# mourisl/Rcorrector

Measured on AMD Instinct MI355X. Metric: corrected reads/sec (150 bp, k=23), higher is better.
Workload: dtype u8/int32/u64

## Files before the change

### include/rcorrector_amd.h

```cpp
#ifndef RCORRECTOR_AMD_H
#define RCORRECTOR_AMD_H

#include <stddef.h>
#include <stdint.h>

#ifdef __cplusplus
extern "C" {
#endif

typedef struct rc_ctx rc_ctx;

typedef enum {
    RC_STATUS_OK = 0,
    RC_STATUS_ARG = -1,
    RC_STATUS_HIP = -2,
    RC_STATUS_IO = -3,
    RC_STATUS_STATE = -4,
    RC_STATUS_NOMEM = -5,
    RC_STATUS_NOSPACE = -6
} rc_status;

typedef struct {
    int device;
    int k;
// ... 189 lines not shown

typedef struct {
    int mode;
    uint32_t n_reads;
    uint64_t nbytes;
    int32_t max_read_len;
    uint8_t *d_seq;
    const uint8_t *d_qual;
    const uint32_t *d_off;
    int32_t *d_ret, *d_l, *d_m, *d_h;
} rc_device_batch;
int rc_correct_device(rc_ctx *ctx, const rc_device_batch *b);
int rc_strong_threshold_device(rc_ctx *ctx, const uint8_t *d_seq, const uint32_t *d_off, uint32_t n_reads,
                               uint64_t nbytes, int32_t max_read_len, int32_t *d_strong);
int rc_strong_threshold_read(rc_ctx *ctx, const char *seq, int32_t *strong);
int rc_correct_read(rc_ctx *ctx, char *seq, const char *qual, int32_t pair_strong_threshold, int32_t *ret);
int rc_kmer_info_read(rc_ctx *ctx, const char *seq, int32_t *l, int32_t *m, int32_t *h);
int rc_probe_device(rc_ctx *ctx, const uint8_t *d_seq, uint64_t nbytes, int32_t *d_counts);
int rc_sync(rc_ctx *ctx);

int rc_profile_enable(rc_ctx *ctx, int on);
int rc_profile_correct_counters(rc_ctx *ctx, uint64_t *reads_listed, uint64_t *gather_rounds, uint64_t *bucket_requests);
int rc_profile_read_rounds(rc_ctx *ctx, int32_t *d_rounds);
int rc_profile_get(rc_ctx *ctx, int kernel, double *total_ms, uint64_t *launches);
int rc_profile_reset(rc_ctx *ctx);

int rc_selftest_get_bound(rc_ctx *ctx, const int32_t *c, size_t n, double error_rate, int32_t *out_int, double *out_dbl);

int rc_debug_routes(rc_ctx *ctx, uint8_t *cls_out, uint8_t *cand_out, uint64_t *runs_out, uint32_t n);

int rc_summary(const rc_ctx *ctx, uint64_t *total_reads, uint64_t *total_corrections);

#ifdef __cplusplus
}
#endif
#endif
```

### rcorrector_amd/binding.py

```python
import ctypes as C
import os
import subprocess

import numpy as np

HERE = os.path.dirname(os.path.abspath(__file__))
CSRC = os.path.join(HERE, "csrc")

ABI_SYMBOLS = [
    "rc_create", "rc_destroy", "rc_last_error", "rc_device_numa_node", "rc_device_memory",
    "rc_table_build", "rc_table_build_device", "rc_table_load_jfdump",
    "rc_table_count_begin", "rc_table_count_add", "rc_table_count_add_device", "rc_table_count_finish",
    "rc_table_count_keep", "rc_table_count_arenas", "rc_table_count_release", "rc_table_count_park", "rc_table_count_finish_sharded", "rc_submit_resident", "rc_wait_resident",
    "rc_table_count_reads_device", "rc_table_write_jfdump", "rc_table_share", "rc_table_replicate", "rc_table_replicate_async", "rc_table_lookup", "rc_table_export", "rc_table_digest", "rc_table_layout", "rc_table_stats",
    "rc_table_count_spectrum", "rc_table_spectrum",
    "rc_recount_begin", "rc_recount_add", "rc_recount_add_device", "rc_recount_follow", "rc_recount_finish",
    "rc_change_report_begin", "rc_change_report_get", "rc_change_report_end",
    "rc_weak_profile_device", "rc_weak_profile_into",
    "rc_dup_census_begin", "rc_dup_census_get", "rc_dup_census_end", "rc_read_keys_device", "rc_dup_census_merge",
    "rc_trust_profile_device", "rc_trust_profile_begin", "rc_trust_profile_get", "rc_trust_profile_end",
    "rc_mate_overlap_device", "rc_mate_overlap_begin", "rc_mate_overlap_get", "rc_mate_overlap_end",
    "rc_estimate_error_rate", "rc_bad_quality_from_hist", "rc_set_run_params", "rc_set_quality_bits", "rc_pack_quality_bits",
    "rc_correct_batch", "rc_set_slot_lanes", "rc_runtime_prepare", "rc_submit", "rc_wait", "rc_host_alloc", "rc_host_free", "rc_host_register", "rc_host_unregister", "rc_correct_batch_traced", "rc_correct_device", "rc_strong_threshold_device", "rc_probe_device", "rc_sync",
    "rc_strong_threshold_read", "rc_correct_read", "rc_kmer_info_read",
    "rc_pack_bases", "rc_submit_packed", "rc_wait_packed", "rc_apply_fixes",
    "rc_profile_enable", "rc_profile_get", "rc_profile_reset", "rc_profile_correct_counters", "rc_profile_read_rounds", "rc_selftest_get_bound", "rc_debug_routes", "rc_summary",
]


class RcorrectorError(RuntimeError):
    pass


def library_path():
    return os.environ.get("RC_LIB") or os.path.join(HERE, "librcorrector_amd.so")


def build_library(quiet=True):
    subprocess.run(["make", "-C", CSRC, "-j4", "all"], check=True,
                   stdout=subprocess.DEVNULL if quiet else None)
    return library_path()


class _Config(C.Structure):
    _fields_ = [("device", C.c_int), ("k", C.c_int), ("max_fix_per_k", C.c_int)]


class _Batch(C.Structure):
    _fields_ = [("mode", C.c_int), ("n", C.c_size_t),
# ... 182 lines not shown
    L.rc_correct_batch.argtypes = [vp, C.POINTER(_Batch)]
    L.rc_submit.argtypes = [vp, C.POINTER(_Batch), C.c_int]
    L.rc_wait.argtypes = [vp, C.c_int]
    L.rc_host_alloc.argtypes = [vp, sz, C.POINTER(C.c_void_p)]
    L.rc_host_free.argtypes = [vp, vp]
    L.rc_correct_device.argtypes = [vp, C.POINTER(_DeviceBatch)]
    L.rc_probe_device.argtypes = [vp, vp, C.c_uint64, vp]
    L.rc_strong_threshold_device.argtypes = [vp, vp, vp, C.c_uint32, C.c_uint64, C.c_int32, vp]
    L.rc_sync.argtypes = [vp]
    L.rc_strong_threshold_read.argtypes = [vp, C.c_char_p, C.POINTER(C.c_int32)]
    L.rc_correct_read.argtypes = [vp, C.c_char_p, C.c_char_p, C.c_int32, C.POINTER(C.c_int32)]
    L.rc_kmer_info_read.argtypes = [vp, C.c_char_p, C.POINTER(C.c_int32), C.POINTER(C.c_int32), C.POINTER(C.c_int32)]
    L.rc_pack_bases.restype = sz
    L.rc_pack_bases.argtypes = [vp, sz, sz, vp, vp, vp, sz]
    L.rc_submit_packed.argtypes = [vp, C.POINTER(_PackedBatch), C.c_int]
    L.rc_wait_packed.argtypes = [vp, C.c_int]
    L.rc_apply_fixes.restype = None
    L.rc_apply_fixes.argtypes = [vp, vp, vp, sz]
    L.rc_profile_enable.argtypes = [vp, C.c_int]
    L.rc_profile_get.argtypes = [vp, C.c_int, C.POINTER(C.c_double), C.POINTER(C.c_uint64)]
    L.rc_profile_reset.argtypes = [vp]
    L.rc_profile_correct_counters.argtypes = [vp, C.POINTER(C.c_uint64), C.POINTER(C.c_uint64), C.POINTER(C.c_uint64)]
    L.rc_profile_read_rounds.argtypes = [vp, vp]
    L.rc_selftest_get_bound.argtypes = [vp, vp, sz, C.c_double, vp, vp]
    L.rc_debug_routes.argtypes = [vp, vp, vp, vp, C.c_uint32]
    L.rc_summary.argtypes = [vp, C.POINTER(C.c_uint64), C.POINTER(C.c_uint64)]
    _lib = L
    return L


def runtime_prepare(hw_queues=16):
    return load_library().rc_runtime_prepare(int(hw_queues))


def pack_reads(seqs):
    lens = np.fromiter((len(s) for s in seqs), dtype=np.int64, count=len(seqs))
    off = np.zeros(len(seqs) + 1, dtype=np.uint32)
    np.cumsum(lens + 1, out=off[1:])
    if seqs:
        arena = np.frombuffer(b"\0".join(seqs) + b"\0", dtype=np.uint8).copy()
    else:
        arena = np.zeros(0, np.uint8)
    return arena, off


def unpack_reads(arena, off):
# ... 443 lines not shown

    def kmer_info_read(self, seq):
        l, m, h = C.c_int32(0), C.c_int32(0), C.c_int32(0)
        self._ck(self._L.rc_kmer_info_read(self._h, bytes(seq), C.byref(l), C.byref(m), C.byref(h)))
        return l.value, m.value, h.value

    def probe_device(self, d_seq, nbytes, d_counts):
        self._ck(self._L.rc_probe_device(self._h, _ptr(d_seq), nbytes, _ptr(d_counts)))

    def sync(self):
        self._ck(self._L.rc_sync(self._h))

    def profile(self, on=True):
        self._ck(self._L.rc_profile_enable(self._h, int(on)))

    def profile_correct_counters(self):
        a, b, c = C.c_uint64(0), C.c_uint64(0), C.c_uint64(0)
        self._ck(self._L.rc_profile_correct_counters(self._h, C.byref(a), C.byref(b), C.byref(c)))
        return a.value, b.value, c.value

    def profile_read_rounds(self, d_rounds=None):
        self._ck(self._L.rc_profile_read_rounds(self._h, None if d_rounds is None else d_rounds.data_ptr()))

    def profile_reset(self):
        self._ck(self._L.rc_profile_reset(self._h))

    def profile_get(self, kernel):
        ms, n = C.c_double(0), C.c_uint64(0)
        self._ck(self._L.rc_profile_get(self._h, kernel, C.byref(ms), C.byref(n)))
        return ms.value, n.value

    def selftest_get_bound(self, c, error_rate):
        c = np.ascontiguousarray(c, dtype=np.int32)
        oi = np.zeros(len(c), dtype=np.int32)
        od = np.zeros(len(c), dtype=np.float64)
        self._ck(self._L.rc_selftest_get_bound(self._h, c.ctypes.data, len(c), error_rate, oi.ctypes.data, od.ctypes.data))
        return oi, od

    def debug_routes(self, n):
        cls, cand, runs = np.zeros(n, np.uint8), np.zeros(n, np.uint8), np.zeros(n, np.uint64)
        self._ck(self._L.rc_debug_routes(self._h, cls.ctypes.data, cand.ctypes.data, runs.ctypes.data, n))
        return cls, cand, runs

    def summary(self):
        a, b = C.c_uint64(0), C.c_uint64(0)
        self._ck(self._L.rc_summary(self._h, C.byref(a), C.byref(b)))
# ... 2 lines not shown
```

### rcorrector_amd/csrc/rc_api.hip

```cpp
#include "rc_api_internal.h"
#include <mutex>

static thread_local char g_create_err[512];

void rc_set_error(rc_ctx *ctx, const char *fmt, ...)
{
    va_list ap;
    va_start(ap, fmt);
    vsnprintf(ctx ? ctx->err : g_create_err, 512, fmt, ap);
    va_end(ap);
}

int rc_dbuf_reserve(rc_ctx *ctx, rc_dbuf *b, size_t bytes)
{
    if (bytes <= b->bytes) return RC_OK;
    if (b->p) {
        RC_CHECK_HIP(ctx, hipStreamSynchronize(ctx->stream));
        (void)hipFree(b->p);
        b->p = nullptr;
        b->bytes = 0;
    }
    size_t want = bytes + bytes / 8 + 256;
    RC_CHECK_HIP(ctx, hipMalloc(&b->p, want));
    b->bytes = want;
// ... 99 lines not shown
        ln->is_lane = true;
        ln->lane_parent = ctx;
    }
    if (refresh) {
        ln->d_buckets = ctx->d_buckets;
        ln->buckets_borrowed = true;
        ln->nb_home = ctx->nb_home;
        ln->layout = ctx->layout;
        ln->ext = ctx->ext;
        ln->nb_alloc = ctx->nb_alloc;
        ln->n_entries = ctx->n_entries;
        ln->table_bytes = ctx->table_bytes;
        ln->filter_words = ctx->filter_words;
        ln->filter_kind = ctx->filter_kind;
        ln->filter_all = ctx->filter_all;
        ln->P = ctx->P;
        ln->params_set = ctx->params_set;
        ln->qual_bits = ctx->qual_bits;
        ln->kept.arenas = ctx->kept.arenas;
        ln->profile = ctx->profile;
        ln->phase_prof = ctx->phase_prof;
        ln->phase_prof_print = ctx->phase_prof_print;
        ln->rounds_out = ctx->rounds_out;
    }
    ctx->slot_home[slot] = ln;
    return ln;
}

int rc_runtime_prepare(int hw_queues)
{
    if (hw_queues < 1) return -1;
    if (getenv("GPU_MAX_HW_QUEUES")) return 0;
    char v[16];
    snprintf(v, sizeof v, "%d", hw_queues);
    return setenv("GPU_MAX_HW_QUEUES", v, 0) == 0 ? 1 : -1;
}

rc_ctx *rc_create(const rc_config *cfg, char *errbuf, size_t errbuf_len)
{
    auto fail = [&](const char *msg) -> rc_ctx * {
        if (errbuf && errbuf_len) snprintf(errbuf, errbuf_len, "%s", msg);
        return nullptr;
    };
    if (!cfg) return fail("rc_create: null config");
    if (cfg->k < 1 || cfg->k > 32) return fail("rc_create: k must be in 1..32 (run_rcorrector.pl:225-228)");
    int ndev = 0;
// ... 188 lines not shown
    if (!ctx) return RC_ERR_ARG;
    uint64_t a = ctx->k3_listed, b = ctx->k3_rounds, c = ctx->k3_requests;
    for (rc_ctx *ln : ctx->lane) {
        if (!ln) continue;
        a += ln->k3_listed;
        b += ln->k3_rounds;
        c += ln->k3_requests;
    }
    if (reads_listed) *reads_listed = a;
    if (gather_rounds) *gather_rounds = b;
    if (bucket_requests) *bucket_requests = c;
    return RC_OK;
}

int rc_profile_read_rounds(rc_ctx *ctx, int32_t *d_rounds)
{
    if (!ctx) return RC_ERR_ARG;
    ctx->rounds_out = d_rounds;
    for (rc_ctx *ln : ctx->lane)
        if (ln) ln->rounds_out = d_rounds;
    return RC_OK;
}

int rc_selftest_get_bound(rc_ctx *ctx, const int32_t *c, size_t n, double error_rate, int32_t *out_int, double *out_dbl)
{
    if (!ctx || (n && (!c || !out_int || !out_dbl))) return RC_ERR_ARG;
    if (n == 0) return RC_OK;
    RC_CHECK_HIP(ctx, hipSetDevice(ctx->device));
    rc_dev_tmp b_c, b_i, b_d;
    RC_CHECK_HIP(ctx, b_c.alloc(n * 4));
    RC_CHECK_HIP(ctx, b_i.alloc(n * 4));
    RC_CHECK_HIP(ctx, b_d.alloc(n * 8));
    RC_CHECK_HIP(ctx, hipMemcpyAsync(b_c.p, c, n * 4, hipMemcpyHostToDevice, ctx->stream));
    int rc = rc_launch_selftest_bound(ctx, b_c.as<int32_t>(), n, error_rate, b_i.as<int32_t>(), b_d.as<double>());
    if (rc) return rc;
    RC_CHECK_HIP(ctx, hipMemcpyAsync(out_int, b_i.p, n * 4, hipMemcpyDeviceToHost, ctx->stream));
    RC_CHECK_HIP(ctx, hipMemcpyAsync(out_dbl, b_d.p, n * 8, hipMemcpyDeviceToHost, ctx->stream));
    RC_CHECK_HIP(ctx, hipStreamSynchronize(ctx->stream));
    return RC_OK;
}

int rc_debug_routes(rc_ctx *ctx, uint8_t *cls_out, uint8_t *cand_out, uint64_t *runs_out, uint32_t n)
{
    if (!ctx || !cls_out || !cand_out || !runs_out) return RC_ERR_ARG;
    const char *why = nullptr;
    if (ctx->routes_state == rc_ctx::RC_ROUTES_NONE)
// ... 49 lines not shown
```

### rcorrector_amd/csrc/rc_correct.hip

```cpp
#include "rc_correct_kernel.h"


#define RC_K2_PF 4
__global__ __launch_bounds__(64) void k_threshold(rc_kernel_args A)
{
    extern __shared__ __attribute__((aligned(16))) uint8_t lds[];
    const rc_lds_layout L = rc_layout(A.cap);
    rc_read_state S;
    rc_carve(lds, L, S);
    DevWave w;
    w.lane = threadIdx.x;
    w.T = A.T;
    w.k = A.P.k;
    w.stack = nullptr;
    const int lane = w.lane, k = A.P.k;
    const uint32_t G = gridDim.x;
    uint32_t r = blockIdx.x;
    if (r >= A.n) return;
    uint32_t o_cur = A.off[r], e_cur = A.off[r + 1];
    uint32_t o_nxt = 0, e_nxt = 0;
    if (r + G < A.n) {
        o_nxt = A.off[r + G];
        e_nxt = A.off[r + G + 1];
    }
// ... 389 lines not shown
    A.worklist = nullptr;
    A.work_stride = 0;
    A.n_work = nullptr;
    A.ret = a.ret;
    A.l = a.l;
    A.m = a.m;
    A.h = a.h;
    A.stack = nullptr;
    A.stack_frames = 0;
    A.work = (uint32_t *)ctx->work.p;
    A.cap = rc_cap_for(a.max_len);
    {
        const int need_seg = (a.max_len + 1) / (ctx->k + 1) + 1;
        int cls = A.cap <= 192 ? 192 : (A.cap <= 320 ? 320 : 1024);
        while (cls < 1024 && rc_seg_capacity(cls) < need_seg) cls = cls == 192 ? 320 : 1024;
        if (rc_seg_capacity(cls) < need_seg) {
            rc_set_error(ctx, "correct: reads of %d bases with k = %d are not supported (too many segments)", a.max_len, ctx->k);
            return RC_ERR_ARG;
        }
        A.cap_class = cls;
    }
    A.phase_cycles = nullptr;
    A.rounds_out = ctx->phase_prof ? ctx->rounds_out : nullptr;
    A.trace = nullptr;
    A.trace_cap = 0;
    A.fused_front_end = a.mode == 0 && !ctx->thr_ready;
    A.tier_lo = a.tier_lo;
    A.tier_hi = a.tier_hi;
    A.pair_override = a.pair_override;
    return RC_OK;
}

static int rc_short_ec(const rc_ctx *ctx, int max_len, int k)
{
    if (max_len > 160) return 0;
    const int kcnt = max_len - k + 1;
    const int ec = kcnt <= 128 ? 8 : (kcnt <= 144 ? 9 : 10);
    return ec < ctx->env_force_ec ? ctx->env_force_ec : ec;
}

int rc_launch_threshold(rc_ctx *ctx, const rc_device_batch_args &a, bool classify)
{
    ctx->cls_ready = false;
    ctx->cand_ready = false;
    if (a.n == 0) return RC_OK;
    rc_kernel_args A;
// ... 230 lines not shown
    else if (A.cap_class == 192)
        hipLaunchKernelGGL((k_correct<192, false, false>), dim3(grid), dim3(64), 0, ctx->stream, A);
    else if (A.cap_class == 320)
        hipLaunchKernelGGL((k_correct<320, false, false>), dim3(grid), dim3(64), 0, ctx->stream, A);
    else
        hipLaunchKernelGGL((k_correct<1024, false, false>), dim3(grid), dim3(64), 0, ctx->stream, A);
    rc_timer_end(ctx, RC_T_CORRECT);
    if (ctx->phase_prof) {
        unsigned long long pc[34];
        uint32_t nwork = a.n, nsec[RC_WORK_CLASSES] = {0};
        RC_CHECK_HIP(ctx, hipMemcpyAsync(pc, A.phase_cycles, sizeof pc, hipMemcpyDeviceToHost, ctx->stream));
        if (A.n_work) RC_CHECK_HIP(ctx, hipMemcpyAsync(nsec, A.n_work, sizeof nsec, hipMemcpyDeviceToHost, ctx->stream));
        RC_CHECK_HIP(ctx, hipStreamSynchronize(ctx->stream));
        if (A.n_work) {
            nwork = 0;
            for (int i = 0; i < RC_WORK_CLASSES; ++i) nwork += nsec[i];
        }
        static const char *names[8] = {"dequeue+load", "polya", "islands/segments", "search", "lower-thresholds", "post-filters", "apply+kmerinfo", "store"};
        unsigned long long tot = 0;
        for (int i = 0; i < 8; ++i) tot += pc[i];
        ctx->k3_listed += nwork;
        ctx->k3_rounds += pc[11];
        ctx->k3_requests += pc[13];
        if (ctx->phase_prof_print) {
        fprintf(stderr, "[rc phase prof] k_correct, %u reads, cycles/read:", a.n);
        for (int i = 0; i < 8; ++i) fprintf(stderr, " %s=%.0f(%.0f%%)", names[i], (double)pc[i] / a.n, 100.0 * pc[i] / (tot ? tot : 1));
        fprintf(stderr, "\n[rc phase prof] work list %u of %u reads; queue empty at %.2f ms, last wave done at %.2f ms; gather rounds: %.2f per listed read, worst read %llu\n",
                nwork, a.n, (double)(pc[9] - pc[8]) / 1e5, (double)(pc[10] - pc[8]) / 1e5, (double)pc[11] / (nwork ? nwork : 1), pc[12]);
        fprintf(stderr, "[rc phase prof] k-mers looked up by the searches: %.1f per listed read, %.1f %% of them not in the table\n",
                (double)pc[14] / (nwork ? nwork : 1), 100.0 * (double)pc[15] / (double)(pc[14] ? pc[14] : 1));
        fprintf(stderr, "[rc phase prof] bucket reads: %.1f per listed read; work-list sections (first to last): %u / %u / %u / %u reads\n",
                (double)pc[13] / (nwork ? nwork : 1), nsec[0], nsec[1], nsec[2], nsec[3]);
        static const char *sn[8] = {"node entry+pop", "refill (gather round)", "keep-run", "single node", "gap windows", "jump", "terminal", "-"};
        fprintf(stderr, "[rc phase prof] inside the search, cycles/read:");
        for (int i = 0; i < 7; ++i) fprintf(stderr, " %s=%.0f", sn[i], (double)pc[16 + i] / a.n);
        fprintf(stderr, "\n");
        const double R = (double)(pc[11] ? pc[11] : 1), KR = (double)(pc[24] ? pc[24] : 1);
        fprintf(stderr, "[rc phase prof] a gather round: %.1f probes, %.1f %% with alternative chains (%.2f walked per round, %.0f %% of them to the end); a keep-run (%.2f per round) keeps %.2f of the %.2f cached nodes it is offered; gap-window rounds %.3f per round (%.1f probes)\n",
                (double)pc[32] / R, 100.0 * (double)pc[33] / R, (double)pc[30] / R, 100.0 * (double)pc[31] / (double)(pc[30] ? pc[30] : 1), KR / R, (double)pc[25] / KR,
                (double)pc[26] / KR, (double)pc[28] / R, (double)pc[29] / (double)(pc[28] ? pc[28] : 1));
        }
    }
    RC_CHECK_HIP(ctx, hipGetLastError());
    return RC_OK;
}

// ... 41 lines not shown
```

### rcorrector_amd/csrc/rc_correct_core.h

```cpp
#pragma once
#include "rc_common.h"

#define RC_BS_INLINE 16
#define RC_K(P) (W::KT > 0 ? W::KT : (P).k)

struct rc_run_params {
    int k;
    int max_fix_per_k;
    double error_rate;
    int bad_qual;
    uint32_t bs[RC_BS_INLINE];
    int flags;
    const uint32_t *bs_ext;
    const uint8_t *bound_small;
};
#define RC_BOUND_SMALL 4096
RC_HD uint32_t rc_bs_lookup(const rc_run_params &P, int t)
{
    if (!P.bs[0] || t < 2) return 0;
    if (t < RC_BS_INLINE) return P.bs[t];
    if (!P.bs_ext || t >= RC_BOUND_STEPS) return 0;
    const uint32_t v = P.bs_ext[t];
    return v == RC_BOUND_NEVER ? 0 : v;
}
// ... 2 lines not shown
struct rc_island {
    short from, to;
};
struct rc_segment {
    short from, to, lanchor, ranchor;
    int top2[2];
};

struct rc_cnt4 {
    int c0, c1, c2, c3;
};

struct rc_frame {
    uint64_t code;
    int inv;
    int pos;
    int t;
    int threshold;
    int fix_cnt;
    int bottleneck;
    rc_cnt4 cnt;
    int mask;
};

struct rc_read_state {
    unsigned char *base;
    int *counts;
    int *v;
    signed char *path;
    signed char *best;
    unsigned char *strongb;
    unsigned char *polya;
    signed char *qual;
    rc_island *isl;
    rc_segment *seg;
    uint64_t *m_a, *m_t;
    uint64_t *m_n, *m_inv;
    uint64_t *m_x;
    uint32_t *pk;
    int *spec_cnt;
    int *spec_meta;
    int *memo;
    uint64_t *spec_code;
    int *spec_inv;
    int *spec_ret;
    int *spec_keep;
// ... 1272 lines not shown
```

### rcorrector_amd/csrc/rc_correct_kernel.h

```cpp
#pragma once
#include <cstddef>
#include <cstdio>
#include <cstdlib>

#include "rc_internal.h"
#include "rc_device.h"

template <bool PROF, bool TRACE = false, bool SORT_REGS = true, int KT_ = 0>
struct DevWaveT {
    static const int STRIDE = 64;
    static constexpr int KT = KT_;
    int lane;
    unsigned long long t_last = 0;
    int cur_phase = 0;
    unsigned long long *acc = nullptr;
#ifdef RC_EXP_ROUNDS
    int rounds = 0;
    __device__ __forceinline__ void stat(int i, int v)
    {
        if (i == 3) rounds += v;
    }
#else
    int rounds = 0, rounds_max = 0;
    long long rounds_sum = 0;
    long long stv[10] = {0, 0, 0, 0, 0, 0, 0, 0, 0, 0};
    __device__ __forceinline__ void stat(int i, int v)
    {
        if (PROF && i == 3) rounds += v;
        if (PROF && i != 3 && i < 10) stv[i] += v;
    }
// ... 29 lines not shown
                int32_t *e = tr + 2 + (size_t)it * RC_TRACE_WORDS;
                for (int c = 0; c < RC_MAX_READ_LENGTH / 64; ++c) {
                    const uint64_t m = ballot64(c << 6, len, [&](int q) { return strongb[q] != 0; });
                    if (lane == 0) {
                        e[4 + 2 * c] = (int32_t)(uint32_t)m;
                        e[5 + 2 * c] = (int32_t)(uint32_t)(m >> 32);
                    }
                }
                if (lane == 0) e[2] = 1;
            }
            sync();
        }
    }
    __device__ __forceinline__ int uni(int x) { return __builtin_amdgcn_readfirstlane(x); }
    __device__ __forceinline__ uint64_t uni64(uint64_t x)
    {
        const uint32_t lo = (uint32_t)__builtin_amdgcn_readfirstlane((int)(uint32_t)x);
        const uint32_t hi = (uint32_t)__builtin_amdgcn_readfirstlane((int)(uint32_t)(x >> 32));
        return ((uint64_t)hi << 32) | lo;
    }
    __device__ __forceinline__ void phase(int id)
    {
        if (id < 8) asm volatile("" : "+v"(lane));
        if (PROF) {
            unsigned long long t = __builtin_readcyclecounter();
            if (lane == 0) acc[cur_phase] += t - t_last;
            t_last = t;
            cur_phase = id;
        }
    }
    rc_table_view T;
    int k;
    rc_frame *stack;

    __device__ __forceinline__ void sync()
    {
        __builtin_amdgcn_fence(__ATOMIC_RELEASE, "wavefront");
        __builtin_amdgcn_wave_barrier();
        __builtin_amdgcn_fence(__ATOMIC_ACQUIRE, "wavefront");
    }

    template <class F>
    __device__ __forceinline__ uint64_t ballot64(int base, int n, F pred)
    {
        const int i = base + lane;
        bool p = false;
// ... 129 lines not shown
        int n2 = 1;
        while (n2 < n) n2 <<= 1;
        for (int i = n + lane; i < n2; i += 64) a[i] = 2147483647;
        sync();
        for (int size = 2; size <= n2; size <<= 1) {
            for (int stride = size >> 1; stride > 0; stride >>= 1) {
                for (int t = lane; t < (n2 >> 1); t += 64) {
                    const int pos = 2 * t - (t & (stride - 1));
                    const int par = pos + stride;
                    const bool up = (pos & size) == 0;
                    const int x = a[pos], y = a[par];
                    if ((x > y) == up) {
                        a[pos] = y;
                        a[par] = x;
                    }
                }
                sync();
            }
        }
    }

    uint32_t *lstack = nullptr;
    int lstack_n = 0;
    static constexpr int FRAME_DWORDS = (int)(sizeof(rc_frame) / 4);
    __device__ __forceinline__ void stack_push(int sp, const rc_frame &f)
    {
        if (sp < lstack_n) {
            if (lane == 0) {
                uint32_t *d = lstack + sp * FRAME_DWORDS;
                d[0] = (uint32_t)f.code;
                d[1] = (uint32_t)(f.code >> 32);
                d[2] = (uint32_t)f.inv;
                d[3] = (uint32_t)f.pos;
                d[4] = (uint32_t)f.t;
                d[5] = (uint32_t)f.threshold;
                d[6] = (uint32_t)f.fix_cnt;
                d[7] = (uint32_t)f.bottleneck;
                d[8] = (uint32_t)f.cnt.c0;
                d[9] = (uint32_t)f.cnt.c1;
                d[10] = (uint32_t)f.cnt.c2;
                d[11] = (uint32_t)f.cnt.c3;
                d[12] = (uint32_t)f.mask;
            }
            sync();
            return;
        }
        if (lane == 0) stack[sp] = f;
        __threadfence_block();
    }
    __device__ __forceinline__ void stack_top(int idx, rc_frame &f)
    {
        static_assert(sizeof(rc_frame) == 56 && offsetof(rc_frame, mask) == 48, "rc_frame layout");
        uint32_t d[13];
        if (idx < lstack_n) {
            const uint32_t *p = lstack + idx * FRAME_DWORDS;
#pragma unroll
            for (int q = 0; q < 13; ++q) d[q] = p[q];
        } else {
            const uint32_t *p = reinterpret_cast<const uint32_t *>(stack + idx);
#pragma unroll
            for (int q = 0; q < 13; ++q) d[q] = __hip_atomic_load(p + q, __ATOMIC_RELAXED, __HIP_MEMORY_SCOPE_WORKGROUP);
        }
        f.code = ((uint64_t)(uint32_t)uni((int)d[1]) << 32) | (uint32_t)uni((int)d[0]);
        f.inv = uni((int)d[2]);
        f.pos = uni((int)d[3]);
        f.t = uni((int)d[4]);
        f.threshold = uni((int)d[5]);
        f.fix_cnt = uni((int)d[6]);
        f.bottleneck = uni((int)d[7]);
        f.cnt.c0 = uni((int)d[8]);
        f.cnt.c1 = uni((int)d[9]);
        f.cnt.c2 = uni((int)d[10]);
        f.cnt.c3 = uni((int)d[11]);
        f.mask = uni((int)d[12]);
    }
    __device__ __forceinline__ void stack_set_mask(int idx, int mask)
    {
        if (idx < lstack_n) {
            if (lane == 0) lstack[idx * FRAME_DWORDS + 12] = (uint32_t)mask;
            sync();
            return;
        }
        if (lane == 0) stack[idx].mask = mask;
        __threadfence_block();
    }
};
typedef DevWaveT<false> DevWave;

#ifndef RC_DEQUEUE
#define RC_DEQUEUE 8
#endif
#define RC_META_WORDS 6

struct rc_lds_layout {
    int cap, cap2;
    size_t o_counts, o_v, o_isl, o_seg, o_base, o_path, o_best, o_strongb, o_polya, o_qual, o_masks, o_spec, o_pk, o_meta, total;
    int mask_words;
};

static __host__ __device__ constexpr inline int rc_seg_capacity(int cap) { return cap <= 192 ? 20 : cap / 6 + 4; }

static __host__ __device__ constexpr inline rc_lds_layout rc_layout(int cap)
{
    rc_lds_layout L{};
    L.cap = cap;
    int c2 = 64;
    while (c2 < cap) c2 <<= 1;
    L.cap2 = c2;
    const int nseg = rc_seg_capacity(cap);
    const int nisl = cap / 3 + 2;
    size_t o = 0;
    L.mask_words = cap / 64 + 2;
    L.o_masks = o;
    o += (size_t)L.mask_words * 8 * 5;
// ... 74 lines not shown
    uint32_t qual_split, qual_base2;
    const uint32_t *off;
    const int32_t *counts;
    int32_t *strong, *info;
    uint8_t *cls;
    uint8_t *cand;
    uint2 *runs;
    const uint32_t *worklist;
    const uint32_t *n_work;
    int32_t *ret, *l, *m, *h;
    rc_frame *stack;
    int stack_frames;
    uint32_t *work;
    int cap;
    int cap_class;
    unsigned long long *phase_cycles;
    int32_t *rounds_out;
    uint32_t work_stride;
    int fused_front_end;
    int32_t *trace;
    int trace_cap;
    int tier_lo, tier_hi;
    int pair_override;
};
__device__ __forceinline__ int rc_unit_max_len(const rc_kernel_args &A, uint32_t r, int len)
{
    if (A.mode == 0) return len;
    const uint32_t half = A.n >> 1, mr = A.mode == 1 ? (r < half ? r + half : r - half) : (r ^ 1u);
    const int ml = (int)(A.off[mr + 1] - A.off[mr]) - 1;
    return ml > len ? ml : len;
}
__device__ __forceinline__ bool rc_in_tier(const rc_kernel_args &A, int unit_max_len) { return unit_max_len > A.tier_lo && unit_max_len <= A.tier_hi; }

template <class W>
__device__ __forceinline__ void rc_load_read(W &w, const rc_kernel_args &A, rc_read_state &S, uint32_t o, int len, int lane, bool with_qual)
{
    S.len = len;
    S.kcnt = len >= RC_K(A.P) ? len - RC_K(A.P) + 1 : 0;
    for (int i = lane; i < len; i += 64) {
        S.base[i] = (unsigned char)rc_base_code(A.seq[o + i]);
        S.counts[i] = i < S.kcnt ? A.counts[o + i] : 0;
        if (with_qual) S.qual[i] = rc_qual_at(A.qual, A.qual_bits, A.qual_split, A.qual_base2, o + (uint32_t)i);
    }
    w.sync();
    rc_build_masks(w, S);
    rc_pack_read(w, S);
// ... 24 lines not shown
    w.lane = threadIdx.x;
    w.tr_cap = A.trace_cap;
    if (PROF) {
        w.acc = reinterpret_cast<unsigned long long *>(lds + L.total);
        if (w.lane < 16) w.acc[w.lane] = 0;
        w.sync();
        w.t_last = __builtin_readcyclecounter();
    }
    w.T = A.T;
    if (TL != 0) w.T.layout = 1;
    if (TL == 1) w.T.ext = 0;
    if (KT != 0) w.T.k = KT;
    w.k = A.P.k;
    w.stack = A.stack + (size_t)blockIdx.x * A.stack_frames;
    w.lstack = reinterpret_cast<uint32_t *>(S.v);
    w.lstack_n = (int)((size_t)L.cap2 * 4 / sizeof(rc_frame));
    if (PROF && w.lane == 0) atomicMin(A.phase_cycles + 8, (unsigned long long)wall_clock64());
    const int n_sections = A.n_work ? RC_WORK_CLASSES : 1;
    int section = 0;
    uint32_t n_work = A.n_work ? (uint32_t)__builtin_amdgcn_readfirstlane((int)A.n_work[0]) : A.n;
    const uint32_t *list = A.worklist;
    uint32_t *heads = A.work;
    uint32_t chunk_lo = 0, chunk_hi = 0, chunk_base = 0;
    uint32_t *meta = reinterpret_cast<uint32_t *>(lds + L.o_meta);
    int head = (int)(blockIdx.x % RC_HEADS), heads_done = 0;
    for (;;) {
        if (chunk_lo >= chunk_hi) {
            bool got = false;
            for (;;) {
                while (heads_done < RC_HEADS) {
                    const uint32_t lo = (uint32_t)(((uint64_t)n_work * (uint32_t)head) / RC_HEADS);
                    const uint32_t hi = (uint32_t)(((uint64_t)n_work * (uint32_t)(head + 1)) / RC_HEADS);
                    uint32_t r0 = hi - lo;
                    if (hi > lo) {
                        if (w.lane == 0) r0 = atomicAdd(heads + head * 32, (uint32_t)RC_DEQUEUE);
                        r0 = (uint32_t)__builtin_amdgcn_readfirstlane((int)r0);
                    }
                    if (r0 < hi - lo) {
                        chunk_lo = lo + r0;
                        chunk_hi = hi - chunk_lo > (uint32_t)RC_DEQUEUE ? chunk_lo + RC_DEQUEUE : hi;
                        got = true;
                        break;
                    }
                    head = head + 1 == RC_HEADS ? 0 : head + 1;
                    ++heads_done;
                }
                if (got || ++section >= n_sections) break;
                n_work = (uint32_t)__builtin_amdgcn_readfirstlane((int)A.n_work[section]);
                list = A.worklist + (size_t)section * A.work_stride;
                heads = A.work + section * (RC_HEADS * 32);
                head = (int)(blockIdx.x % RC_HEADS);
                heads_done = 0;
            }
            if (!got) {
                if (PROF && w.lane == 0) atomicMin(A.phase_cycles + 9, (unsigned long long)wall_clock64());
                break;
            }
            chunk_base = chunk_lo;
            if ((uint32_t)w.lane < chunk_hi - chunk_lo) {
                uint32_t ri = chunk_lo + (uint32_t)w.lane;
                if (list) ri = list[ri];
                uint32_t *mw = meta + w.lane * RC_META_WORDS;
                mw[0] = ri;
                mw[1] = A.off[ri];
                mw[2] = A.off[ri + 1];
                if (!A.fused_front_end) {
                    mw[3] = (uint32_t)A.strong[ri];
                    mw[4] = (uint32_t)A.info[ri];
                    if (A.mode == 1) {
                        const uint32_t half = A.n >> 1;
                        mw[5] = (uint32_t)A.strong[ri < half ? ri + half : ri - half];
                    } else if (A.mode == 2)
                        mw[5] = (uint32_t)A.strong[ri ^ 1u];
                }
            }
            w.sync();
        }
        const int ci = (int)(chunk_lo - chunk_base);
        ++chunk_lo;
        const uint32_t *me = meta + ci * RC_META_WORDS;
        const uint32_t r = (uint32_t)w.uni((int)me[0]);
        const uint32_t o = (uint32_t)w.uni((int)me[1]);
        w.phase(0);
        if (TRACE) {
            w.tr = A.trace + (size_t)r * (2 + (size_t)A.trace_cap * RC_TRACE_WORDS);
            if (w.lane == 0) w.tr[0] = w.tr[1] = 0;
            w.sync();
        }
#if defined(RC_EXP_STOP) && RC_EXP_STOP == 0
        if (w.lane == 0) A.ret[r] = (int)o;
        continue;
#endif
        rc_load_read(w, A, S, o, w.uni((int)(me[2] - o) - 1), w.lane, true);
#if defined(RC_EXP_STOP) && RC_EXP_STOP == 1
        if (w.lane == 0) A.ret[r] = (int)S.m_inv[0] + (int)S.pk[1] + S.counts[5] + S.qual[7];
        w.sync();
        continue;
#endif
        int strong0, info0;
        if (A.fused_front_end) {
            w.phase(1);
            strong0 = rc_front_end(w, S, A.P, &info0);
        } else {
            strong0 = w.uni((int)me[3]);
            info0 = w.uni((int)me[4]);
        }
// ... 23 lines not shown
                }
            }
            w.sync();
            rc_pack_read(w, S);
        }
        int l, m, h;
        rc_kmer_info(w, S, A.P, ret, &l, &m, &h);
        if (w.lane == 0) {
            A.ret[r] = ret;
#ifdef RC_EXP_ROUNDS
            A.l[r] = w.rounds;
            w.rounds = 0;
#else
            A.l[r] = l;
#endif
            A.m[r] = m;
            A.h[r] = h;
        }
        w.sync();
        w.phase(7);
#ifndef RC_EXP_ROUNDS
        if (PROF) {
            if (A.rounds_out && w.lane == 0) A.rounds_out[r] = w.rounds;
            w.rounds_sum += w.rounds;
            w.rounds_max = w.rounds > w.rounds_max ? w.rounds : w.rounds_max;
            w.rounds = 0;
        }
#endif
    }
    if (PROF && w.lane == 0) {
        w.phase(7);
        for (int i = 0; i < 8; ++i) atomicAdd(A.phase_cycles + i, w.acc[i]);
        for (int i = 8; i < 16; ++i) atomicAdd(A.phase_cycles + 8 + i, w.acc[i]);
        atomicMax(A.phase_cycles + 10, (unsigned long long)wall_clock64());
#ifndef RC_EXP_ROUNDS
        atomicAdd(A.phase_cycles + 11, (unsigned long long)w.rounds_sum);
        atomicMax(A.phase_cycles + 12, (unsigned long long)w.rounds_max);
        for (int i = 0; i < 10; ++i)
            if (i != 3) atomicAdd(A.phase_cycles + 24 + i, (unsigned long long)w.stv[i]);
#endif
    }
    if (PROF) {
        const int req = w.reduce_add((int)w.n_req), prb = w.reduce_add((int)w.n_probe), abs_ = w.reduce_add((int)w.n_absent);
        if (w.lane == 0) {
            atomicAdd(A.phase_cycles + 13, (unsigned long long)(uint32_t)req);
            atomicAdd(A.phase_cycles + 14, (unsigned long long)(uint32_t)prb);
// ... 13 lines not shown
```

### rcorrector_amd/csrc/rc_internal.h

```cpp
#pragma once
#include <hip/hip_runtime.h>
#include <stddef.h>
#include <stdint.h>

#include <atomic>
#include <mutex>
#include <type_traits>
#include <utility>
#include <vector>

#include "rc_correct_core.h"

#define RC_CHECK_HIP(ctx, expr)                                                                  \
    do {                                                                                         \
        hipError_t _e = (expr);                                                                  \
        if (_e != hipSuccess) {                                                                  \
            rc_set_error((ctx), "%s failed: %s (%s:%d)", #expr, hipGetErrorString(_e), __FILE__, \
                         __LINE__);                                                              \
            return RC_ERR_HIP;                                                                   \
        }                                                                                        \
    } while (0)

enum { RC_OK = 0, RC_ERR_ARG = -1, RC_ERR_HIP = -2, RC_ERR_IO = -3, RC_ERR_STATE = -4, RC_ERR_NOMEM = -5, RC_ERR_NOSPACE = -6 };

// ... 64 lines not shown
    bool rep_staged = false;
    void drop(int parts, bool free_bufs);
    void reset() { drop(RC_OBS_ALL, false); }
};

struct rc_kernel_timer {
    double ms = 0;
    uint64_t launches = 0;
};

enum { RC_T_PROBE = 0, RC_T_THRESH = 1, RC_T_CORRECT = 2, RC_T_SINGLE = 3, RC_T_WEAK = 4, RC_T_TRUST_PLANES = 5, RC_T_TRUST = 6, RC_T_COUNT };

struct rc_ctx {
    int device = 0;
    int k = 23;
    int n_cu = 256;
    hipStream_t stream = nullptr;
    hipEvent_t ev0 = nullptr, ev1 = nullptr;
    bool profile = false;
    bool phase_prof = false;
    bool phase_prof_print = false;
    uint64_t k3_listed = 0, k3_rounds = 0, k3_requests = 0;
    int32_t *rounds_out = nullptr;
    rc_kernel_timer timers[RC_T_COUNT];

    rc_run_params P;
    bool params_set = false;
    bool qual_bits = false;
    rc_ctx *lane[4] = {nullptr, nullptr, nullptr, nullptr};
    rc_ctx *slot_home[4] = {nullptr, nullptr, nullptr, nullptr};
    bool is_lane = false;
    bool env_slot_lanes = true;

    uint32_t *d_buckets = nullptr;
    bool buckets_borrowed = false;
    uint32_t nb_home = 0;
    double table_load = 0.50;
    bool table_load_set = false;
    double table_load_packed = 0.50;
    int layout = 0;
    int ext = 0;
    int layout_pref = 1;
    uint32_t nb_alloc = 0;
    size_t n_entries = 0;
    size_t table_bytes = 0;
    void *counted_codes = nullptr;
// ... 201 lines not shown
```

Baseline: 364.4 million.

## Taper dequeue chunks near queue end and drop fences on far-stack pushes

Each wave now takes a ticket from the work-head atomic and maps it to a chunk: full-size chunks at first, then single reads for the last gridDim.x items, so the work at the tail is spread more evenly across waves. The workgroup fence after every far-memory stack push or mask write becomes conditional (off by default), and a fence is issued only before reading a far frame. The change also adds per-read timing and profiling records behind PROF, plus new API calls to read them. The tapered tail raises the number of atomics per read near the end, and deferring the fence relies on the read-side fence for ordering.

```diff
diff --git a/include/rcorrector_amd.h b/include/rcorrector_amd.h
--- a/include/rcorrector_amd.h
+++ b/include/rcorrector_amd.h
@@ -235,6 +235,8 @@
 int rc_profile_enable(rc_ctx *ctx, int on);
 int rc_profile_correct_counters(rc_ctx *ctx, uint64_t *reads_listed, uint64_t *gather_rounds, uint64_t *bucket_requests);
 int rc_profile_read_rounds(rc_ctx *ctx, int32_t *d_rounds);
+int rc_profile_read_records(rc_ctx *ctx, uint32_t *d_records);
+int rc_profile_correct_clocks(rc_ctx *ctx, uint64_t *first_wave_in, uint64_t *queue_empty, uint64_t *last_wave_out);
 int rc_profile_get(rc_ctx *ctx, int kernel, double *total_ms, uint64_t *launches);
 int rc_profile_reset(rc_ctx *ctx);
 
diff --git a/rcorrector_amd/binding.py b/rcorrector_amd/binding.py
--- a/rcorrector_amd/binding.py
+++ b/rcorrector_amd/binding.py
@@ -24,7 +24,7 @@
     "rc_correct_batch", "rc_set_slot_lanes", "rc_runtime_prepare", "rc_submit", "rc_wait", "rc_host_alloc", "rc_host_free", "rc_host_register", "rc_host_unregister", "rc_correct_batch_traced", "rc_correct_device", "rc_strong_threshold_device", "rc_probe_device", "rc_sync",
     "rc_strong_threshold_read", "rc_correct_read", "rc_kmer_info_read",
     "rc_pack_bases", "rc_submit_packed", "rc_wait_packed", "rc_apply_fixes",
-    "rc_profile_enable", "rc_profile_get", "rc_profile_reset", "rc_profile_correct_counters", "rc_profile_read_rounds", "rc_selftest_get_bound", "rc_debug_routes", "rc_summary",
+    "rc_profile_enable", "rc_profile_get", "rc_profile_reset", "rc_profile_correct_counters", "rc_profile_read_rounds", "rc_profile_read_records", "rc_profile_correct_clocks", "rc_selftest_get_bound", "rc_debug_routes", "rc_summary",
 ]
 
 
@@ -253,6 +253,9 @@
     L.rc_profile_reset.argtypes = [vp]
     L.rc_profile_correct_counters.argtypes = [vp, C.POINTER(C.c_uint64), C.POINTER(C.c_uint64), C.POINTER(C.c_uint64)]
     L.rc_profile_read_rounds.argtypes = [vp, vp]
+    if hasattr(L, "rc_profile_read_records"):
+        L.rc_profile_read_records.argtypes = [vp, vp]
+        L.rc_profile_correct_clocks.argtypes = [vp, C.POINTER(C.c_uint64), C.POINTER(C.c_uint64), C.POINTER(C.c_uint64)]
     L.rc_selftest_get_bound.argtypes = [vp, vp, sz, C.c_double, vp, vp]
     L.rc_debug_routes.argtypes = [vp, vp, vp, vp, C.c_uint32]
     L.rc_summary.argtypes = [vp, C.POINTER(C.c_uint64), C.POINTER(C.c_uint64)]
@@ -742,6 +745,14 @@
     def profile_read_rounds(self, d_rounds=None):
         self._ck(self._L.rc_profile_read_rounds(self._h, None if d_rounds is None else d_rounds.data_ptr()))
 
+    def profile_read_records(self, d_records=None):
+        self._ck(self._L.rc_profile_read_records(self._h, None if d_records is None else d_records.data_ptr()))
+
+    def profile_correct_clocks(self):
+        a, b, c = C.c_uint64(), C.c_uint64(), C.c_uint64()
+        self._ck(self._L.rc_profile_correct_clocks(self._h, C.byref(a), C.byref(b), C.byref(c)))
+        return a.value, b.value, c.value
+
     def profile_reset(self):
         self._ck(self._L.rc_profile_reset(self._h))
 
diff --git a/rcorrector_amd/csrc/rc_api.hip b/rcorrector_amd/csrc/rc_api.hip
--- a/rcorrector_amd/csrc/rc_api.hip
+++ b/rcorrector_amd/csrc/rc_api.hip
@@ -145,6 +145,7 @@
         ln->phase_prof = ctx->phase_prof;
         ln->phase_prof_print = ctx->phase_prof_print;
         ln->rounds_out = ctx->rounds_out;
+        ln->records_out = ctx->records_out;
     }
     ctx->slot_home[slot] = ln;
     return ln;
@@ -379,6 +380,24 @@
     return RC_OK;
 }
 
+int rc_profile_read_records(rc_ctx *ctx, uint32_t *d_records)
+{
+    if (!ctx) return RC_ERR_ARG;
+    ctx->records_out = d_records;
+    for (rc_ctx *ln : ctx->lane)
+        if (ln) ln->records_out = d_records;
+    return RC_OK;
+}
+
+int rc_profile_correct_clocks(rc_ctx *ctx, uint64_t *first_wave_in, uint64_t *queue_empty, uint64_t *last_wave_out)
+{
+    if (!ctx) return RC_ERR_ARG;
+    if (first_wave_in) *first_wave_in = ctx->k3_clock[0];
+    if (queue_empty) *queue_empty = ctx->k3_clock[1];
+    if (last_wave_out) *last_wave_out = ctx->k3_clock[2];
+    return RC_OK;
+}
+
 int rc_selftest_get_bound(rc_ctx *ctx, const int32_t *c, size_t n, double error_rate, int32_t *out_int, double *out_dbl)
 {
     if (!ctx || (n && (!c || !out_int || !out_dbl))) return RC_ERR_ARG;
diff --git a/rcorrector_amd/csrc/rc_correct.hip b/rcorrector_amd/csrc/rc_correct.hip
--- a/rcorrector_amd/csrc/rc_correct.hip
+++ b/rcorrector_amd/csrc/rc_correct.hip
@@ -435,6 +435,7 @@
     }
     A.phase_cycles = nullptr;
     A.rounds_out = ctx->phase_prof ? ctx->rounds_out : nullptr;
+    A.records_out = ctx->phase_prof ? ctx->records_out : nullptr;
     A.trace = nullptr;
     A.trace_cap = 0;
     A.fused_front_end = a.mode == 0 && !ctx->thr_ready;
@@ -711,6 +712,7 @@
         ctx->k3_listed += nwork;
         ctx->k3_rounds += pc[11];
         ctx->k3_requests += pc[13];
+        for (int i = 0; i < 3; ++i) ctx->k3_clock[i] = pc[8 + i];
         if (ctx->phase_prof_print) {
         fprintf(stderr, "[rc phase prof] k_correct, %u reads, cycles/read:", a.n);
         for (int i = 0; i < 8; ++i) fprintf(stderr, " %s=%.0f(%.0f%%)", names[i], (double)pc[i] / a.n, 100.0 * pc[i] / (tot ? tot : 1));
diff --git a/rcorrector_amd/csrc/rc_correct_core.h b/rcorrector_amd/csrc/rc_correct_core.h
--- a/rcorrector_amd/csrc/rc_correct_core.h
+++ b/rcorrector_amd/csrc/rc_correct_core.h
@@ -48,6 +48,49 @@
     rc_cnt4 cnt;
     int mask;
 };
+
+template <class B>
+RC_HD void rc_stack_push(B &b, int sp, const rc_frame &f)
+{
+    if (sp < b.lstack_n)
+        b.lds_put(sp, f);
+    else
+        b.far_put(sp, f);
+}
+template <class B>
+RC_HD void rc_stack_top(B &b, int idx, rc_frame &f)
+{
+    if (idx < b.lstack_n) {
+        b.lds_get(idx, f);
+    } else {
+        b.far_wait();
+        b.far_get(idx, f);
+    }
+}
+template <class B>
+RC_HD void rc_stack_set_mask(B &b, int idx, int mask)
+{
+    if (idx < b.lstack_n)
+        b.lds_put_mask(idx, mask);
+    else
+        b.far_put_mask(idx, mask);
+}
+
+RC_HD bool rc_dequeue_chunk(uint32_t len, uint32_t waves, uint32_t per, uint32_t t, uint32_t *lo, uint32_t *hi)
+{
+    const uint32_t tail = len < waves ? len : waves;
+    const uint32_t nfull = (len - tail) / per;
+    if (t < nfull) {
+        *lo = t * per;
+        *hi = *lo + per;
+        return true;
+    }
+    const uint32_t e = nfull * per + (t - nfull);
+    if (t - nfull >= len - nfull * per) return false;
+    *lo = e;
+    *hi = e + 1;
+    return true;
+}
 
 struct rc_read_state {
     unsigned char *base;
diff --git a/rcorrector_amd/csrc/rc_correct_kernel.h b/rcorrector_amd/csrc/rc_correct_kernel.h
--- a/rcorrector_amd/csrc/rc_correct_kernel.h
+++ b/rcorrector_amd/csrc/rc_correct_kernel.h
@@ -6,6 +6,9 @@
 #include "rc_internal.h"
 #include "rc_device.h"
 
+#ifndef RC_K3_PUSH_WAIT
+#define RC_K3_PUSH_WAIT 0
+#endif
 template <bool PROF, bool TRACE = false, bool SORT_REGS = true, int KT_ = 0>
 struct DevWaveT {
     static const int STRIDE = 64;
@@ -81,6 +84,7 @@
     __device__ __forceinline__ void phase(int id)
     {
         if (id < 8) asm volatile("" : "+v"(lane));
+        if (PROF && id == 8) ++visits;
         if (PROF) {
             unsigned long long t = __builtin_readcyclecounter();
             if (lane == 0) acc[cur_phase] += t - t_last;
@@ -256,45 +260,37 @@
 
     uint32_t *lstack = nullptr;
     int lstack_n = 0;
+    int visits = 0, deepest = 0, far_pushes = 0;
     static constexpr int FRAME_DWORDS = (int)(sizeof(rc_frame) / 4);
-    __device__ __forceinline__ void stack_push(int sp, const rc_frame &f)
-    {
-        if (sp < lstack_n) {
-            if (lane == 0) {
-                uint32_t *d = lstack + sp * FRAME_DWORDS;
-                d[0] = (uint32_t)f.code;
-                d[1] = (uint32_t)(f.code >> 32);
-                d[2] = (uint32_t)f.inv;
-                d[3] = (uint32_t)f.pos;
-                d[4] = (uint32_t)f.t;
-                d[5] = (uint32_t)f.threshold;
-                d[6] = (uint32_t)f.fix_cnt;
-                d[7] = (uint32_t)f.bottleneck;
-                d[8] = (uint32_t)f.cnt.c0;
-                d[9] = (uint32_t)f.cnt.c1;
-                d[10] = (uint32_t)f.cnt.c2;
-                d[11] = (uint32_t)f.cnt.c3;
-                d[12] = (uint32_t)f.mask;
-            }
-            sync();
-            return;
-        }
+    __device__ __forceinline__ void lds_put(int sp, const rc_frame &f)
+    {
+        if (lane == 0) {
+            uint32_t *d = lstack + sp * FRAME_DWORDS;
+            d[0] = (uint32_t)f.code;
+            d[1] = (uint32_t)(f.code >> 32);
+            d[2] = (uint32_t)f.inv;
+            d[3] = (uint32_t)f.pos;
+            d[4] = (uint32_t)f.t;
+            d[5] = (uint32_t)f.threshold;
+            d[6] = (uint32_t)f.fix_cnt;
+            d[7] = (uint32_t)f.bottleneck;
+            d[8] = (uint32_t)f.cnt.c0;
+            d[9] = (uint32_t)f.cnt.c1;
+            d[10] = (uint32_t)f.cnt.c2;
+            d[11] = (uint32_t)f.cnt.c3;
+            d[12] = (uint32_t)f.mask;
+        }
+        sync();
+    }
+    __device__ __forceinline__ void far_put(int sp, const rc_frame &f)
+    {
         if (lane == 0) stack[sp] = f;
-        __threadfence_block();
-    }
-    __device__ __forceinline__ void stack_top(int idx, rc_frame &f)
-    {
-        static_assert(sizeof(rc_frame) == 56 && offsetof(rc_frame, mask) == 48, "rc_frame layout");
-        uint32_t d[13];
-        if (idx < lstack_n) {
-            const uint32_t *p = lstack + idx * FRAME_DWORDS;
-#pragma unroll
-            for (int q = 0; q < 13; ++q) d[q] = p[q];
-        } else {
-            const uint32_t *p = reinterpret_cast<const uint32_t *>(stack + idx);
-#pragma unroll
-            for (int q = 0; q < 13; ++q) d[q] = __hip_atomic_load(p + q, __ATOMIC_RELAXED, __HIP_MEMORY_SCOPE_WORKGROUP);
-        }
+        if (PROF) ++far_pushes;
+        if (RC_K3_PUSH_WAIT) __threadfence_block();
+    }
+    __device__ __forceinline__ void far_wait() { __threadfence_block(); }
+    __device__ __forceinline__ void unpack(const uint32_t (&d)[13], rc_frame &f)
+    {
         f.code = ((uint64_t)(uint32_t)uni((int)d[1]) << 32) | (uint32_t)uni((int)d[0]);
         f.inv = uni((int)d[2]);
         f.pos = uni((int)d[3]);
@@ -308,22 +304,50 @@
         f.cnt.c3 = uni((int)d[11]);
         f.mask = uni((int)d[12]);
     }
-    __device__ __forceinline__ void stack_set_mask(int idx, int mask)
-    {
-        if (idx < lstack_n) {
-            if (lane == 0) lstack[idx * FRAME_DWORDS + 12] = (uint32_t)mask;
-            sync();
-            return;
-        }
+    __device__ __forceinline__ void lds_get(int idx, rc_frame &f)
+    {
+        static_assert(sizeof(rc_frame) == 56 && offsetof(rc_frame, mask) == 48, "rc_frame layout");
+        uint32_t d[13];
+        const uint32_t *p = lstack + idx * FRAME_DWORDS;
+#pragma unroll
+        for (int q = 0; q < 13; ++q) d[q] = p[q];
+        unpack(d, f);
+    }
+    __device__ __forceinline__ void far_get(int idx, rc_frame &f)
+    {
+        uint32_t d[13];
+        const uint32_t *p = reinterpret_cast<const uint32_t *>(stack + idx);
+#pragma unroll
+        for (int q = 0; q < 13; ++q) d[q] = __hip_atomic_load(p + q, __ATOMIC_RELAXED, __HIP_MEMORY_SCOPE_WORKGROUP);
+        unpack(d, f);
+    }
+    __device__ __forceinline__ void lds_put_mask(int idx, int mask)
+    {
+        if (lane == 0) lstack[idx * FRAME_DWORDS + 12] = (uint32_t)mask;
+        sync();
+    }
+    __device__ __forceinline__ void far_put_mask(int idx, int mask)
+    {
         if (lane == 0) stack[idx].mask = mask;
-        __threadfence_block();
-    }
+        if (RC_K3_PUSH_WAIT) __threadfence_block();
+    }
+    __device__ __forceinline__ void stack_push(int sp, const rc_frame &f)
+    {
+        if (PROF) deepest = sp > deepest ? sp : deepest;
+        rc_stack_push(*this, sp, f);
+    }
+    __device__ __forceinline__ void stack_top(int idx, rc_frame &f) { rc_stack_top(*this, idx, f); }
+    __device__ __forceinline__ void stack_set_mask(int idx, int mask) { rc_stack_set_mask(*this, idx, mask); }
 };
 typedef DevWaveT<false> DevWave;
 
+#ifndef RC_K3_TAPER
+#define RC_K3_TAPER 1
+#endif
 #ifndef RC_DEQUEUE
 #define RC_DEQUEUE 8
 #endif
+#define RC_K3_RECORD_WORDS 12
 #define RC_META_WORDS 6
 
 struct rc_lds_layout {
@@ -444,6 +468,7 @@
     int trace_cap;
     int tier_lo, tier_hi;
     int pair_override;
+    uint32_t *records_out;
 };
 __device__ __forceinline__ int rc_unit_max_len(const rc_kernel_args &A, uint32_t r, int len)
 {
@@ -514,6 +539,7 @@
     const uint32_t *list = A.worklist;
     uint32_t *heads = A.work;
     uint32_t chunk_lo = 0, chunk_hi = 0, chunk_base = 0;
+    unsigned long long t_dequeue = 0, t_start = 0;
     uint32_t *meta = reinterpret_cast<uint32_t *>(lds + L.o_meta);
     int head = (int)(blockIdx.x % RC_HEADS), heads_done = 0;
     for (;;) {
@@ -523,16 +549,16 @@
                 while (heads_done < RC_HEADS) {
                     const uint32_t lo = (uint32_t)(((uint64_t)n_work * (uint32_t)head) / RC_HEADS);
                     const uint32_t hi = (uint32_t)(((uint64_t)n_work * (uint32_t)(head + 1)) / RC_HEADS);
-                    uint32_t r0 = hi - lo;
                     if (hi > lo) {
-                        if (w.lane == 0) r0 = atomicAdd(heads + head * 32, (uint32_t)RC_DEQUEUE);
-                        r0 = (uint32_t)__builtin_amdgcn_readfirstlane((int)r0);
-                    }
-                    if (r0 < hi - lo) {
-                        chunk_lo = lo + r0;
-                        chunk_hi = hi - chunk_lo > (uint32_t)RC_DEQUEUE ? chunk_lo + RC_DEQUEUE : hi;
-                        got = true;
-                        break;
+                        uint32_t t = 0, c0, c1;
+                        if (w.lane == 0) t = atomicAdd(heads + head * 32, 1u);
+                        t = (uint32_t)__builtin_amdgcn_readfirstlane((int)t);
+                        if (rc_dequeue_chunk(hi - lo, RC_K3_TAPER ? gridDim.x : 0u, RC_DEQUEUE, t, &c0, &c1)) {
+                            chunk_lo = lo + c0;
+                            chunk_hi = lo + c1;
+                            got = true;
+                            break;
+                        }
                     }
                     head = head + 1 == RC_HEADS ? 0 : head + 1;
                     ++heads_done;
@@ -549,6 +575,7 @@
                 break;
             }
             chunk_base = chunk_lo;
+            if (PROF) t_dequeue = (unsigned long long)wall_clock64();
             if ((uint32_t)w.lane < chunk_hi - chunk_lo) {
                 uint32_t ri = chunk_lo + (uint32_t)w.lane;
                 if (list) ri = list[ri];
@@ -574,6 +601,7 @@
         const uint32_t r = (uint32_t)w.uni((int)me[0]);
         const uint32_t o = (uint32_t)w.uni((int)me[1]);
         w.phase(0);
+        if (PROF) t_start = (unsigned long long)wall_clock64();
         if (TRACE) {
             w.tr = A.trace + (size_t)r * (2 + (size_t)A.trace_cap * RC_TRACE_WORDS);
             if (w.lane == 0) w.tr[0] = w.tr[1] = 0;
@@ -643,6 +671,23 @@
 #ifndef RC_EXP_ROUNDS
         if (PROF) {
             if (A.rounds_out && w.lane == 0) A.rounds_out[r] = w.rounds;
+            if (A.records_out && w.lane == 0) {
+                const unsigned long long t_end = (unsigned long long)wall_clock64();
+                uint32_t *rec = A.records_out + (size_t)r * RC_K3_RECORD_WORDS;
+                rec[0] = (uint32_t)t_dequeue;
+                rec[1] = (uint32_t)(t_dequeue >> 32);
+                rec[2] = (uint32_t)t_start;
+                rec[3] = (uint32_t)(t_start >> 32);
+                rec[4] = (uint32_t)t_end;
+                rec[5] = (uint32_t)(t_end >> 32);
+                rec[6] = (uint32_t)section;
+                rec[7] = blockIdx.x;
+                rec[8] = (uint32_t)w.visits;
+                rec[9] = (uint32_t)w.deepest;
+                rec[10] = (uint32_t)w.far_pushes;
+                rec[11] = (uint32_t)w.rounds;
+            }
+            w.visits = w.deepest = w.far_pushes = 0;
             w.rounds_sum += w.rounds;
             w.rounds_max = w.rounds > w.rounds_max ? w.rounds : w.rounds_max;
             w.rounds = 0;
diff --git a/rcorrector_amd/csrc/rc_internal.h b/rcorrector_amd/csrc/rc_internal.h
--- a/rcorrector_amd/csrc/rc_internal.h
+++ b/rcorrector_amd/csrc/rc_internal.h
@@ -110,6 +110,8 @@
     bool phase_prof_print = false;
     uint64_t k3_listed = 0, k3_rounds = 0, k3_requests = 0;
     int32_t *rounds_out = nullptr;
+    uint32_t *records_out = nullptr;
+    uint64_t k3_clock[3] = {0, 0, 0};
     rc_kernel_timer timers[RC_T_COUNT];
 
     rc_run_params P;
```

Result: no change. 365.1 million (median of 2 runs) (+0.2%).
